# rapidsai/cugraph-gnn

Hardware: AMD Instinct MI355X
Metric: sampled-edges/sec (sample+renumber+feature-gather+SAGEConv fwd), ogbn-products-like fan-out [25, 10] (higher is better)
Workload: dtype int64 ids (int32 timed as a variant) + f32 features (SAGE lin_l/lin_r product: bf16x3-split MFMA, f32 accumulate); 1 GPU; ogbn-products-like RMAT: V=2449029, E=118462496 directed (CSR row_ptr i64 / col i64 replicated per GPU), feat fp32 [V,100], batch 1024/GPU, fan-out [25, 10], 2-layer SAGEConv(mean) 100-256-47 fwd, step = 8 call groups of 188 mini-batches; parallelism=dp1 (seeds sharded, no data-path collective)

## Files before the change

cugraph-gnn_amd/csrc/wg_rng.hpp:

```cpp
#pragma once
#include <hip/hip_runtime.h>

#include <cstdint>

namespace wgamd {

struct PcgJump {
  uint64_t a;
  uint64_t s;
};

struct PcgJumpTables {
  PcgJump t[4][256];
  constexpr PcgJumpTables() : t{}
  {
    uint64_t base_a = 6364136223846793005ULL, base_s = 1;
    for (int k = 0; k < 4; k++) {
      t[k][0].a = 1;
      t[k][0].s = 0;
      for (int c = 1; c < 256; c++) {
        t[k][c].a = t[k][c - 1].a * base_a;
        t[k][c].s = t[k][c - 1].s * base_a + base_s;
      }
      for (int d = 0; d < 8; d++) {
        uint64_t na = base_a * base_a, ns = base_s * base_a + base_s;
        base_a = na;
        base_s = ns;
      }
    }
  }
};

__device__ __constant__ const PcgJumpTables g_pcg_jump{};

struct Pcg32 {
  uint64_t state;
  uint64_t inc;

  static constexpr uint64_t kMult = 6364136223846793005ULL;

  __host__ __device__ __forceinline__ uint32_t next_u32()
  {
    uint64_t old = state;
    state        = old * kMult + inc;
    uint32_t x   = (uint32_t)(((old >> 18u) ^ old) >> 27u);
    uint32_t rot = (uint32_t)(old >> 59u);
    return (x >> rot) | (x << ((0u - rot) & 31u));
  }

  __host__ __device__ __forceinline__ void skipahead(uint64_t delta)
  {
    uint64_t acc_mult = 1u, acc_plus = 0u, cur_mult = kMult, cur_plus = inc;
    while (delta) {
      if (delta & 1u) {
        acc_mult *= cur_mult;
        acc_plus = acc_plus * cur_mult + cur_plus;
      }
      cur_plus = (cur_mult + 1u) * cur_plus;
      cur_mult *= cur_mult;
      delta >>= 1u;
    }
    state = acc_mult * state + acc_plus;
  }

  __host__ __device__ __forceinline__ Pcg32(uint64_t seed, uint64_t subsequence)
  {
    state = 0u;
    inc   = (subsequence << 1u) | 1u;
    (void)next_u32();
    state += seed;
    (void)next_u32();
    skipahead(subsequence);
  }

  __device__ __forceinline__ void jump_table(uint32_t n)
  {
    PcgJump j = g_pcg_jump.t[0][n & 255u];
#pragma unroll
    for (int k = 1; k < 4; k++) {
      const uint32_t c = (n >> (8 * k)) & 255u;
      if (c) {
        const PcgJump m = g_pcg_jump.t[k][c];
        j.s             = j.s * m.a + m.s;
        j.a             = j.a * m.a;
      }
    }
    state = j.a * state + inc * j.s;
  }

  struct table_tag {};
  __device__ __forceinline__ Pcg32(uint64_t seed, uint32_t subsequence, table_tag, uint32_t extra_draws = 0)
  {
    inc   = ((uint64_t)subsequence << 1u) | 1u;
    state = (inc + seed) * kMult + inc;
    jump_table(subsequence + extra_draws);
  }

  __host__ __device__ __forceinline__ int32_t next_i31() { return (int32_t)(next_u32() & 0x7fffffffu); }
  __host__ __device__ __forceinline__ uint64_t next_u64()
  {
    uint64_t lo = next_u32();
    uint64_t hi = next_u32();
    return lo | (hi << 32u);
  }
  __host__ __device__ __forceinline__ int64_t next_i63() { return (int64_t)(next_u64() & 0x7fffffffffffffffULL); }
  __host__ __device__ __forceinline__ float next_f32() { return (float)(next_u32() >> 8u) / 16777216.0f; }
};

}
```

cugraph-gnn_amd/csrc/wg_sample.hip:

```cpp
#include <algorithm>
#include <cmath>

#include "wg_common.hpp"
#include "wg_rng.hpp"

namespace wgamd {
namespace {

template <typename T>
struct dtype_of;
template <>
struct dtype_of<int32_t> {
  static constexpr wholememory_dtype_t value = WHOLEMEMORY_DT_INT;
};
template <>
struct dtype_of<int64_t> {
  static constexpr wholememory_dtype_t value = WHOLEMEMORY_DT_INT64;
};

__host__ __device__ constexpr int ref_block_threads(int M)
{
  int f = (M - 1) / 32;
  return f < 3 ? 32 : f < 6 ? 64 : f < 12 ? 128 : 256;
}
// ... 102 lines not shown

template <typename ColT>
__device__ __forceinline__ ColT col_at(const ColT* __restrict__ col, int64_t at)
{
  return col ? col[at] : (ColT)0;
}

constexpr int kWalkGrid = 256 * 16;

template <typename ColT>
__device__ __forceinline__ void emit(ColT* dst, int* src_lid, int64_t* edge_gid, int64_t out, ColT v,
                                     int seed_index, int64_t gid)
{
  if (dst) dst[out] = v;
  if (src_lid) src_lid[out] = seed_index;
  if (edge_gid) edge_gid[out] = gid;
}

struct loc_rec {
  int64_t start;
  int i;
  int deg;
  int base;
  int i_local;
  int batch;
  int pad;
};
static_assert(sizeof(loc_rec) == 32, "one 32-byte sector per record");
constexpr int kLocBuckets = 4096;
constexpr int kLocBlocks  = 128;
constexpr int kLocThreads = 1024;

template <typename SeedT>
__global__ void __launch_bounds__(kLocThreads)
locality_hist_kernel(const SeedT* __restrict__ seeds, dev_count n_, int shift, int* __restrict__ hist )
{
  __shared__ int h[kLocBuckets];
  const int n = n_.get(), per = (n + kLocBlocks - 1) / kLocBlocks;
  const int lo = min(n, (int)blockIdx.x * per), hi = min(n, lo + per);
  for (int k = threadIdx.x; k < kLocBuckets; k += kLocThreads) h[k] = 0;
  __syncthreads();
  for (int i = lo + threadIdx.x; i < hi; i += kLocThreads)
    atomicAdd(&h[min((int)((uint64_t)seeds[i] >> shift), kLocBuckets - 1)], 1);
  __syncthreads();
  for (int k = threadIdx.x; k < kLocBuckets; k += kLocThreads) hist[(int64_t)blockIdx.x * kLocBuckets + k] = h[k];
}

template <typename SeedT>
__global__ void __launch_bounds__(kLocThreads)
locality_scatter_kernel(const SeedT* __restrict__ seeds, dev_count n_, int shift, const int* __restrict__ hist,
                        const int64_t* __restrict__ row_start, const int* __restrict__ row_deg, const int* __restrict__ offsets,
                        rng_plan rng, loc_rec* __restrict__ recs)
{
  __shared__ int cursor[kLocBuckets];
  __shared__ int wave_tot[kLocThreads / 64];
  static_assert(kLocBuckets == 4 * kLocThreads, "thread t owns buckets 4 t .. 4 t + 3");
  const int n = n_.get(), per = (n + kLocBlocks - 1) / kLocBlocks;
  const int lo = min(n, (int)blockIdx.x * per), hi = min(n, lo + per);
  int tot[4] = {0, 0, 0, 0}, before[4] = {0, 0, 0, 0};
  const int4* h4 = reinterpret_cast<const int4*>(hist);
  for (int b = 0; b < kLocBlocks; b++) {
    const int4 v = h4[(int64_t)b * (kLocBuckets / 4) + threadIdx.x];
    tot[0] += v.x; tot[1] += v.y; tot[2] += v.z; tot[3] += v.w;
    if (b < (int)blockIdx.x) { before[0] += v.x; before[1] += v.y; before[2] += v.z; before[3] += v.w; }
  }
  const int sum = tot[0] + tot[1] + tot[2] + tot[3];
  int inc = sum;
  const int lane = threadIdx.x & 63, wave = threadIdx.x >> 6;
#pragma unroll
  for (int d = 1; d < 64; d <<= 1) {
    const int up = __shfl_up(inc, d, 64);
    if (lane >= d) inc += up;
  }
  if (lane == 63) wave_tot[wave] = inc;
  __syncthreads();
  int run = inc - sum;
  for (int w = 0; w < wave; w++) run += wave_tot[w];
#pragma unroll
  for (int k = 0; k < 4; k++) {
    cursor[4 * threadIdx.x + k] = run + before[k];
    run += tot[k];
  }
  __syncthreads();
  for (int i = lo + threadIdx.x; i < hi; i += kLocThreads) {
    const int j = atomicAdd(&cursor[min((int)((uint64_t)seeds[i] >> shift), kLocBuckets - 1)], 1);
    loc_rec r;
    r.start = row_start[i];
    r.i     = i;
    r.deg   = row_deg[i];
    r.base  = offsets[i];
    r.i_local = i;
    r.batch   = 0;
    if (rng.target_batch) {
      r.batch   = rng.target_batch[i];
      r.i_local = i - rng.target_seg[r.batch];
    }
    r.pad   = 0;
    recs[j] = r;
  }
}

template <typename SeedT, typename ColT, int LANES>
__global__ void __launch_bounds__(256) sample_uniform_halfwave_kernel(const int64_t* __restrict__ row_ptr,
                                                                      const ColT* __restrict__ col,
                                                                      const SeedT* __restrict__ seeds,
                                                                      dev_count n_,
                                                                      int M,
                                                                      rng_plan rng,
                                                                      const int* __restrict__ offsets,
                                                                      ColT* __restrict__ dst,
                                                                      int* __restrict__ src_lid,
                                                                      int64_t* __restrict__ edge_gid,
                                                                      const int64_t* __restrict__ row_start,
                                                                      const int* __restrict__ row_deg,
                                                                      const loc_rec* __restrict__ recs = nullptr)
{
  const int n    = n_.get();
  const int lane = threadIdx.x & 63;
  const int hl   = lane & (LANES - 1);
  const int hb   = lane & ~(LANES - 1);
  int i          = (int)(((int64_t)blockIdx.x * blockDim.x + threadIdx.x) / LANES);
  loc_rec rec{};
  if (recs) {
    constexpr int kGroups = 256 / LANES;
    const int per_x = ((n + 7) / 8 + kGroups - 1) / kGroups * kGroups;
    const int k     = (int)(blockIdx.x >> 3) * kGroups + (int)threadIdx.x / LANES;
    const int j     = (int)(blockIdx.x & 7) * per_x + k;
    i               = n;
    if (k < per_x && j < n) {
      rec = recs[j];
      i   = rec.i;
    }
  }
  int32_t r_draw = 0;
  if (i < n && hl < M) {
    uint64_t random_seed;
    int i_local;
    if (recs) {
      i_local     = rec.i_local;
      random_seed = rng.seeds_dev ? rng.seeds_dev[rec.batch] : rng.seed;
    } else
      rng.resolve(i, random_seed, i_local);
    if (i_local < (1 << 26)) {
      Pcg32 g(random_seed, (uint32_t)(i_local * 32 + hl), Pcg32::table_tag{});
      r_draw = g.next_i31();
    } else {
      Pcg32 g(random_seed, stream_id(i_local, 32, hl));
      r_draw = g.next_i31();
    }
  }
  int64_t start = 0;
  int N = 0, base = 0;
  if (i < n && recs) {
    start = rec.start;
    N     = rec.deg;
    base  = rec.base;
  } else if (i < n) {
    if (row_start) {
      start = row_start[i];
      N     = row_deg[i];
    } else {
      int64_t nid = (int64_t)seeds[i];
      start       = row_ptr[nid];
      N           = (int)(row_ptr[nid + 1] - start);
    }
    base = offsets[i];
  }
  const bool pick = N > M;
  if (__ballot(pick) == 0ull) {
    if (hl < N) emit<ColT>(dst, src_lid, edge_gid, (int64_t)base + hl, col_at<ColT>(col, start + hl), i, start + hl);
    return;
  }
  int r = 0;
  if (pick && hl < M) r = r_draw % (N - hl);
  const int tail = N - hl - 1;
  int p1 = -1, p2 = -1;
  for (int s = 0; s + 1 < M; s++) {
    const int rs    = __shfl(r, hb | s, 64);
    const bool prev = s < hl;
    p1 = (prev && rs == r) ? s : p1;
    p2 = (prev && rs == tail) ? s : p2;
  }
  int root = p2 >= 0 ? p2 : hl;
#pragma unroll
  for (int round = 0; round < (LANES == 32 ? 5 : 4); round++) root = __shfl(root, hb | root, 64);
  const int val = N - root - 1;
  const int vp1 = __shfl(val, hb | (p1 & (LANES - 1)), 64);
  const int a   = p1 >= 0 ? vp1 : r;
  if (pick) {
    if (hl < M) emit<ColT>(dst, src_lid, edge_gid, (int64_t)base + hl, col_at<ColT>(col, start + a), i, start + a);
  } else if (hl < N) {
    emit<ColT>(dst, src_lid, edge_gid, (int64_t)base + hl, col_at<ColT>(col, start + hl), i, start + hl);
  }
}

template <typename SeedT, typename ColT, int GW, int K, bool EXACT>
__global__ void __launch_bounds__(256)
sample_uniform_multi_kernel(const ColT* __restrict__ col, dev_count n_, int M_rt, rng_plan rng, const int* __restrict__ offsets,
                            ColT* __restrict__ dst, int* __restrict__ src_lid, int64_t* __restrict__ edge_gid,
                            const int64_t* __restrict__ row_start, const int* __restrict__ row_deg,
                            const loc_rec* __restrict__ recs)
{
  constexpr int kGPW    = 64 / GW;
  constexpr int kGroups = 4 * kGPW;
  constexpr int kRounds = GW <= 2 ? 1 : GW <= 4 ? 2 : GW <= 8 ? 3 : GW <= 16 ? 4 : 5;
  const int M    = EXACT ? GW : M_rt;
  const int n    = n_.get();
  const int lane = threadIdx.x & 63;
  const int grp  = lane / GW;
  const int hl   = lane - grp * GW;
  const int hb   = grp * GW;
  const bool live_group = grp < kGPW;
  const int wg_group    = (int)(threadIdx.x >> 6) * kGPW + grp;
  const int per_x = ((n + 7) / 8 + kGroups * K - 1) / (kGroups * K) * (kGroups * K);
  const int64_t n_chunks = recs ? (int64_t)(per_x / (kGroups * K)) * 8 : ((int64_t)n + kGroups * K - 1) / (kGroups * K);
  for (int64_t chunk = blockIdx.x; chunk < n_chunks; chunk += gridDim.x) {
  int i[K], N[K], base[K], i_local[K], batch[K];
  int64_t start[K];
  if (recs) {
    const int k0    = ((int)(chunk >> 3) * kGroups + wg_group) * K;
#pragma unroll
    for (int k = 0; k < K; k++) {
      const int j = (int)(chunk & 7) * per_x + k0 + k;
      i[k] = n, N[k] = 0, base[k] = 0, start[k] = 0, i_local[k] = 0, batch[k] = 0;
      if (live_group && k0 + k < per_x && j < n) {
        const loc_rec r = recs[j];
        i[k] = r.i, N[k] = r.deg, base[k] = r.base, start[k] = r.start, i_local[k] = r.i_local, batch[k] = r.batch;
      }
    }
  } else {
    const int64_t g = chunk * kGroups + wg_group;
#pragma unroll
    for (int k = 0; k < K; k++) {
      i[k] = live_group ? (int)min(g * K + k, (int64_t)n) : n;
      N[k] = 0, base[k] = 0, start[k] = 0, i_local[k] = i[k], batch[k] = 0;
      if (i[k] < n) {
        start[k] = row_start[i[k]];
        N[k]     = row_deg[i[k]];
        base[k]  = offsets[i[k]];
        if (rng.target_batch) batch[k] = rng.target_batch[i[k]];
      }
    }
    if (rng.target_batch) {
#pragma unroll
      for (int k = 0; k < K; k++)
        if (i[k] < n) i_local[k] = i[k] - rng.target_seg[batch[k]];
    }
  }
  int32_t r_draw[K];
#pragma unroll
  for (int k = 0; k < K; k++) {
    r_draw[k] = 0;
    if (i[k] < n && hl < M) {
      const uint64_t random_seed = rng.seeds_dev ? rng.seeds_dev[rng.target_batch ? batch[k] : 0] : rng.seed;
      if (i_local[k] < (1 << 26)) {
        Pcg32 g(random_seed, (uint32_t)(i_local[k] * 32 + hl), Pcg32::table_tag{});
        r_draw[k] = g.next_i31();
      } else {
        Pcg32 g(random_seed, stream_id(i_local[k], 32, hl));
        r_draw[k] = g.next_i31();
      }
    }
  }
  int a[K];
#pragma unroll
  for (int k = 0; k < K; k++) {
    const bool pick = N[k] > M;
    a[k]            = hl;
    if (__ballot(pick) != 0ull) {
      int r = 0;
      if (pick && hl < M) r = r_draw[k] % (N[k] - hl);
      const int tail = N[k] - hl - 1;
      int p1 = -1, p2 = -1;
      auto step = [&](int s) {
        const int rs    = __shfl(r, hb + s, 64);
        const bool prev = s < hl;
        p1 = (prev && rs == r) ? s : p1;
        p2 = (prev && rs == tail) ? s : p2;
      };
      if constexpr (EXACT) {
#pragma unroll
        for (int s = 0; s + 1 < GW; s++) step(s);
      } else {
        for (int s = 0; s + 1 < M; s++) step(s);
      }
      int root = p2 >= 0 ? p2 : hl;
#pragma unroll
      for (int round = 0; round < kRounds; round++) root = __shfl(root, hb + root, 64);
      const int val = N[k] - root - 1;
      const int vp1 = __shfl(val, hb + max(p1, 0), 64);
      if (pick) a[k] = p1 >= 0 ? vp1 : r;
    }
  }
  ColT v[K];
  bool on[K];
#pragma unroll
  for (int k = 0; k < K; k++) {
    on[k] = live_group && hl < (N[k] > M ? M : N[k]);
    v[k]  = on[k] ? col_at<ColT>(col, start[k] + a[k]) : (ColT)0;
  }
#pragma unroll
  for (int k = 0; k < K; k++)
    if (on[k]) emit<ColT>(dst, src_lid, edge_gid, (int64_t)base[k] + hl, v[k], i[k], start[k] + a[k]);
  }
}

constexpr int kHashSlots = 4096;

__device__ __forceinline__ int lds_hash_find(const int* keys, int pos)
{
  uint32_t h = ((uint32_t)pos * 2654435761u) & (kHashSlots - 1);
  while (true) {
    int k = keys[h];
    if (k == pos || k == -1) return (int)h;
    h = (h + 1) & (kHashSlots - 1);
  }
}

template <typename SeedT, typename ColT>
__global__ void __launch_bounds__(256) sample_uniform_block_kernel(const int64_t* __restrict__ row_ptr,
                                                                   const ColT* __restrict__ col,
                                                                   const SeedT* __restrict__ seeds,
                                                                   dev_count n_,
                                                                   int M,
                                                                   int B,
                                                                   int items,
                                                                   rng_plan rng,
                                                                   const int* __restrict__ offsets,
                                                                   ColT* __restrict__ dst,
                                                                   int* __restrict__ src_lid,
                                                                   int64_t* __restrict__ edge_gid)
{
  __shared__ int r[1024];
  __shared__ int a[1024];
  __shared__ int hkeys[kHashSlots];
  __shared__ int hvals[kHashSlots];
  const int i = blockIdx.x;
  if (i >= n_.get()) return;
  const int64_t nid   = (int64_t)seeds[i];
  const int64_t start = row_ptr[nid];
  const int N         = (int)(row_ptr[nid + 1] - start);
  if (N <= 0) return;
  const int base = offsets[i];
  if (N <= M) {
    for (int j = threadIdx.x; j < N; j += blockDim.x)
      emit<ColT>(dst, src_lid, edge_gid, (int64_t)base + j, col_at<ColT>(col, start + j), i, start + j);
    return;
  }
  for (int h = threadIdx.x; h < kHashSlots; h += blockDim.x) hkeys[h] = -1;
  if ((int)threadIdx.x < B) {
    uint64_t random_seed;
    int i_local;
    rng.resolve(i, random_seed, i_local);
    Pcg32 g(random_seed, stream_id(i_local, B, threadIdx.x));
    for (int k = 0; k < items; k++) {
      int id = k * B + threadIdx.x;
      int v  = g.next_i31();
      if (id < M) r[id] = v % (N - id);
    }
  }
  __syncthreads();
  if (threadIdx.x == 0) {
    for (int t = 0; t < M; t++) {
      const int rt = r[t], tail = N - t - 1;
      int s1     = lds_hash_find(hkeys, rt);
      int q_rt   = hkeys[s1] == rt ? hvals[s1] : rt;
      int s2     = lds_hash_find(hkeys, tail);
      int q_tail = hkeys[s2] == tail ? hvals[s2] : tail;
      a[t]       = q_rt;
      hkeys[s1]  = rt;
      hvals[s1]  = q_tail;
    }
  }
  __syncthreads();
  for (int t = threadIdx.x; t < M; t += blockDim.x)
    emit<ColT>(dst, src_lid, edge_gid, (int64_t)base + t, col_at<ColT>(col, start + a[t]), i, start + a[t]);
}

template <typename SeedT, typename ColT>
__global__ void __launch_bounds__(64) sample_uniform_reservoir_kernel(const int64_t* __restrict__ row_ptr,
                                                                      const ColT* __restrict__ col,
                                                                      const SeedT* __restrict__ seeds,
                                                                      dev_count n_,
                                                                      int M,
                                                                      rng_plan rng,
                                                                      const int* __restrict__ offsets,
                                                                      ColT* __restrict__ dst,
                                                                      int* __restrict__ src_lid,
                                                                      int64_t* __restrict__ edge_gid)
{
  const int i = blockIdx.x;
  if (i >= n_.get()) return;
  const int64_t nid   = (int64_t)seeds[i];
  const int64_t start = row_ptr[nid];
  const int N         = (int)(row_ptr[nid + 1] - start);
  if (N <= 0) return;
  const int64_t base = offsets[i];
  if (N <= M) {
    for (int j = threadIdx.x; j < N; j += blockDim.x)
      emit<ColT>(dst, src_lid, edge_gid, base + j, col_at<ColT>(col, start + j), i, start + j);
    return;
  }
  for (int s = threadIdx.x; s < M; s += blockDim.x) dst[base + s] = (ColT)s;
  __syncthreads();
  if (threadIdx.x < 32) {
    uint64_t random_seed;
    int i_local;
    rng.resolve(i, random_seed, i_local);
    Pcg32 g(random_seed, stream_id(i_local, 32, threadIdx.x));
    for (int idx = M + threadIdx.x; idx < N; idx += 32) {
      int rn = g.next_i31() % (idx + 1);
      if (rn < M) {
        if constexpr (sizeof(ColT) == 8)
          atomicMax(reinterpret_cast<long long*>(dst + base + rn), (long long)idx);
        else
          atomicMax(reinterpret_cast<int*>(dst + base + rn), idx);
      }
    }
  }
  __syncthreads();
  for (int s = threadIdx.x; s < M; s += blockDim.x) {
    int sel = (int)__hip_atomic_load(dst + base + s, __ATOMIC_RELAXED, __HIP_MEMORY_SCOPE_AGENT);
    emit<ColT>(dst, src_lid, edge_gid, base + s, col_at<ColT>(col, start + sel), i, start + sel);
  }
}

__device__ __forceinline__ float ares_key(float w, Pcg32& g, bool* redrawn = nullptr)
{
  float u = g.next_f32();
  u       = (float)(-(0.5 + 0.5 * (double)u));
  uint64_t x;
  int zero_draws = -1;
  do {
    x = g.next_u64();
    zero_draws++;
  } while (!x);
  if (redrawn != nullptr && zero_draws > 0) *redrawn = true;
  int one_bit = __clzll((long long)x) + zero_draws * 64;
  u *= exp2f((float)(-one_bit));
#ifdef WG_TUNE_CHEAP_KEY
  return u * 1.442695f * __builtin_amdgcn_rcpf(w);
#endif
  return (log1pf(u) / logf(2.0f)) * (1.0f / w);
}

constexpr int kWaveRowCap = 1024;
static_assert(kWaveRowCap == kWaveRowCapDecl, "keep the two in step");

__device__ __forceinline__ uint32_t key_bits(float k)
{
  uint32_t b = __float_as_uint(k);
  return (b & 0x80000000u) ? ~b : (b | 0x80000000u);
}

constexpr int kLdsKeys = kWeightedLdsKeys;

template <typename SeedT, typename ColT, typename WeightT, int B, int T>
__global__ void __launch_bounds__(T) sample_weighted_kernel(const int64_t* __restrict__ row_ptr,
                                                            const ColT* __restrict__ col,
                                                            const WeightT* __restrict__ weight,
                                                            const SeedT* __restrict__ seeds,
                                                            dev_count n_,
                                                            int M,
                                                            rng_plan rng,
                                                            const int* __restrict__ offsets,
                                                            uint32_t* __restrict__ slab,
                                                            int64_t slab_len,
                                                            ColT* __restrict__ dst,
                                                            int* __restrict__ src_lid,
                                                            int64_t* __restrict__ edge_gid,
                                                            int* __restrict__ lists ,
                                                            int list_cap,
                                                            int redo = 0 )
{
  static_assert(T % B == 0 && T % 64 == 0, "threads must be a multiple of the stream layout and of the wave");
  __shared__ uint32_t lds_keys[kLdsKeys];
  __shared__ int hist[256];
  __shared__ int sh_digit, sh_need, sh_redo;
  __shared__ int wave_cnt[2][T / 64];
  __shared__ int sh_li;
  const int n_live  = n_.get();
  const int n_huge  = lists && !redo ? lists[8] : 0;
  const int count   = lists ? (redo ? lists[kWeightedRedoCount] : n_huge + lists[7]) : n_live;
  uint32_t* gkeys   = slab + (int64_t)blockIdx.x * slab_len;
  int li            = blockIdx.x;
  while (true) {
  __syncthreads();
  if (lists) {
    if (threadIdx.x == 0) sh_li = atomicAdd(lists + (redo ? kWeightedRedoHead : 9), 1);
    __syncthreads();
    li = sh_li;
  }
  if (li >= count) break;
  const int i = lists ? (redo ? lists[kWeightedListHead + (int64_t)kWeightedRedoList * list_cap + li]
                         : li < n_huge ? lists[kWeightedListHead + 8 * (int64_t)list_cap + li]
                                       : lists[kWeightedListHead + 7 * (int64_t)list_cap + (li - n_huge)])
                      : li;
  if (!lists) li += gridDim.x;
  if (i >= n_live) continue;
  uint64_t random_seed;
  int i_rng;
  rng.resolve(i, random_seed, i_rng);
  const int64_t nid   = (int64_t)seeds[i];
  const int64_t start = row_ptr[nid];
  const int N         = (int)(row_ptr[nid + 1] - start);
  if (N <= 0) continue;
  const int64_t base = offsets[i];
  if (M <= 0 || N <= M) {
    for (int j = threadIdx.x; j < N; j += T)
      emit<ColT>(dst, src_lid, edge_gid, base + j, col_at<ColT>(col, start + j), i, start + j);
    continue;
  }
  const bool in_lds = N <= kLdsKeys;
  auto put = [&](int id, uint32_t k) { if (in_lds) lds_keys[id] = k; else gkeys[id] = k; };
  auto get = [&](int id) -> uint32_t {
    return in_lds ? lds_keys[id] : __hip_atomic_load(gkeys + id, __ATOMIC_RELAXED, __HIP_MEMORY_SCOPE_AGENT);
  };
  if (threadIdx.x == 0) sh_redo = 0;
  __syncthreads();
  {
    constexpr int hop = T / B;
    const int lane = threadIdx.x % B, part = threadIdx.x / B;
    const int L     = lane < N ? (N - lane + B - 1) / B : 0;
    const int share = (L + hop - 1) / hop;
    const int m0 = part * share, m1 = min(L, m0 + share);
    bool redrawn = false;
    if (m0 < m1) {
      const int64_t sid = (int64_t)i_rng * B + lane;
      Pcg32 g = (sid < (1ll << 31)) ? Pcg32(random_seed, (uint32_t)sid, Pcg32::table_tag{}, 3u * (uint32_t)m0)
                                    : Pcg32(random_seed, stream_id(i_rng, B, lane));
      if (sid >= (1ll << 31)) g.skipahead(3u * (uint64_t)m0);
      for (int m = m0; m < m1; m++) {
        const int id = lane + m * B;
        put(id, key_bits(ares_key((float)weight[start + id], g, &redrawn)));
      }
    }
    if (redrawn) sh_redo = 1;
  }
  __syncthreads();
  if (T > B && sh_redo) {
    if (threadIdx.x < B) {
      Pcg32 g = stream_generator(random_seed, i_rng, B, threadIdx.x);
      for (int id = threadIdx.x; id < N; id += B) put(id, key_bits(ares_key((float)weight[start + id], g)));
    }
    __syncthreads();
  }
  uint32_t prefix = 0, prefix_mask = 0;
  int need = M;
  for (int shift = 24; shift >= 0; shift -= 8) {
    for (int h = threadIdx.x; h < 256; h += T) hist[h] = 0;
    __syncthreads();
    for (int id = threadIdx.x; id < N; id += T) {
      uint32_t k = get(id);
      if ((k & prefix_mask) == prefix) atomicAdd(&hist[(k >> shift) & 255], 1);
    }
    __syncthreads();
    if (threadIdx.x < 64) {
      const int l  = threadIdx.x;
      const int h0 = hist[4 * l], h1 = hist[4 * l + 1], h2 = hist[4 * l + 2], h3 = hist[4 * l + 3];
      const int own = h0 + h1 + h2 + h3;
      int inc = own;
      for (int off = 1; off < 64; off <<= 1) {
        int v = __shfl_down(inc, off);
        if (l + off < 64) inc += v;
      }
      int acc = inc - own;
      if (acc < need && need <= inc) {
        int d = 4 * l + 3;
        if (acc + h3 < need) {
          acc += h3;
          d = 4 * l + 2;
          if (acc + h2 < need) {
            acc += h2;
            d = 4 * l + 1;
            if (acc + h1 < need) {
              acc += h1;
              d = 4 * l;
            }
          }
        }
        sh_digit = d;
        sh_need  = need - acc;
      }
    }
    __syncthreads();
    prefix |= (uint32_t)sh_digit << shift;
    prefix_mask |= 255u << shift;
    need = sh_need;
    __syncthreads();
  }
  const uint32_t thr = prefix;
  int out_run = 0, tie_run = 0;
  const int lane = threadIdx.x & 63, wave = threadIdx.x >> 6;
  for (int chunk = 0; chunk < N; chunk += T) {
    int id     = chunk + threadIdx.x;
    uint32_t k = id < N ? get(id) : 0u;
    bool gt    = id < N && k > thr;
    bool eq    = id < N && k == thr;
    uint64_t meq = __ballot(eq);
    int eq_before_in_wave = __popcll(meq & ((1ull << lane) - 1ull));
    if (lane == 0) wave_cnt[1][wave] = __popcll(meq);
    __syncthreads();
    int eq_before = tie_run + eq_before_in_wave, eq_total = 0;
    for (int w = 0; w < T / 64; w++) {
      if (w < wave) eq_before += wave_cnt[1][w];
      eq_total += wave_cnt[1][w];
// ... 392 lines not shown
  __shared__ float c_a[kCandCap];
  __shared__ uint32_t c_kb[kCandCap];
  __shared__ int hist[256];
  __shared__ int sh_li, sh_count, sh_rare, sh_digit, sh_need, sh_keep, sh_eq;
  __shared__ uint32_t sh_thr, sh_kmin, sh_sel[2];
  __shared__ uint32_t sh_wthr[W];
  __shared__ int keep_id[32], eq_id[kEqCap];
  __shared__ float keep_a[32], eq_a[kEqCap];
  const int tid = threadIdx.x, lane = tid & 63, wave = tid >> 6;
  const int n_live = n_.get();
  const int n_huge = lists[8];
  const int count  = n_huge + lists[7];

  auto append = [&](int id, float a) {
    const int p = atomicAdd(&sh_count, 1);
    if (p < kCandCap) {
      c_id[p] = id;
      c_a[p]  = a;
    } else {
      sh_rare = 1;
    }
  };

  while (true) {
    __syncthreads();
    if (tid == 0) sh_li = atomicAdd(lists + 9, 1);
    __syncthreads();
    const int li = sh_li;
    if (li >= count) break;
    const int i = li < n_huge ? lists[kWeightedListHead + 8 * (int64_t)list_cap + li]
                              : lists[kWeightedListHead + 7 * (int64_t)list_cap + (li - n_huge)];
    if (i >= n_live) continue;
    uint64_t random_seed;
    int i_rng;
    rng.resolve(i, random_seed, i_rng);
    const int64_t nid   = (int64_t)seeds[i];
    const int64_t start = row_ptr[nid];
    const int N         = (int)(row_ptr[nid + 1] - start);
    const int64_t base  = offsets[i];
    if (tid == 0) {
      sh_count = 0;
      sh_rare  = force_redo;
      sh_thr   = 0x7f800000u;
    }
    auto compress = [&](bool last) {
      __syncthreads();
      const int n = min(sh_count, kCandCap);
      for (int e = tid; e < n; e += T) c_kb[e] = key_bits(ares_key_exact(c_a[e], (float)weight[start + c_id[e]]));
      if (tid == 0) {
        sh_keep = 0;
        sh_eq   = 0;
        sh_kmin = ~0u;
      }
      __syncthreads();
      uint32_t prefix = 0u, hi = 0u;
      int need = M;
      if (n <= 256) {
        if (wave == 0) {
          uint32_t kb[4];
#pragma unroll
          for (int j = 0; j < 4; j++) kb[j] = lane + 64 * j < n ? c_kb[lane + 64 * j] : 0u;
          int match = n;
#pragma unroll 1
          for (int bit = 31; bit >= 0 && match != need; bit--) {
            const uint32_t cand = prefix | (1u << bit);
            hi |= 1u << bit;
            int cnt = 0;
#pragma unroll
            for (int j = 0; j < 4; j++) cnt += __popcll(__ballot(kb[j] != 0u && (kb[j] & hi) == cand));
            if (cnt >= need) {
              prefix = cand;
              match  = cnt;
            } else {
              need -= cnt;
              match -= cnt;
            }
          }
          if (lane == 0) {
            sh_sel[0] = prefix;
            sh_sel[1] = hi;
            sh_need   = need;
          }
        }
        __syncthreads();
        prefix = sh_sel[0];
        hi     = sh_sel[1];
        need   = sh_need;
      } else {
        for (int shift = 24; shift >= 0; shift -= 8) {
          for (int h = tid; h < 256; h += T) hist[h] = 0;
          __syncthreads();
          for (int e = tid; e < n; e += T) {
            const uint32_t kk = c_kb[e];
            if ((kk & hi) == prefix) atomicAdd(&hist[(kk >> shift) & 255], 1);
          }
          __syncthreads();
          if (tid < 64) {
            const int l  = tid;
            const int h0 = hist[4 * l], h1 = hist[4 * l + 1], h2 = hist[4 * l + 2], h3 = hist[4 * l + 3];
            const int own = h0 + h1 + h2 + h3;
            int inc = own;
            for (int off = 1; off < 64; off <<= 1) {
              int v = __shfl_down(inc, off);
              if (l + off < 64) inc += v;
            }
            int acc = inc - own;
            if (acc < need && need <= inc) {
              int d = 4 * l + 3;
              if (acc + h3 < need) {
                acc += h3;
                d = 4 * l + 2;
                if (acc + h2 < need) {
                  acc += h2;
                  d = 4 * l + 1;
                  if (acc + h1 < need) {
                    acc += h1;
                    d = 4 * l;
                  }
                }
              }
              sh_digit = d;
              sh_need  = need - acc;
            }
          }
          __syncthreads();
          prefix |= (uint32_t)sh_digit << shift;
          hi |= 255u << shift;
          need = sh_need;
          __syncthreads();
        }
      }
      for (int e = tid; e < n; e += T) {
        const uint32_t kk = c_kb[e], kd = kk & hi;
        if (kk != 0u && kd > prefix) {
          const int p = atomicAdd(&sh_keep, 1);
          keep_id[p]  = c_id[e];
          keep_a[p]   = c_a[e];
          atomicMin(&sh_kmin, kk);
        } else if (kk != 0u && kd == prefix) {
          const int q = atomicAdd(&sh_eq, 1);
          if (q < kEqCap) {
            eq_id[q] = c_id[e];
            eq_a[q]  = c_a[e];
            atomicMin(&sh_kmin, kk);
          } else {
            sh_rare = 1;
          }
        }
      }
      __syncthreads();
      const int eqc = min(sh_eq, kEqCap);
      if (tid < eqc) {
        int rank = 0;
        for (int j = 0; j < eqc; j++) rank += eq_id[j] < eq_id[tid] ? 1 : 0;
        if (rank < need) {
          const int p = atomicAdd(&sh_keep, 1);
          keep_id[p]  = eq_id[tid];
          keep_a[p]   = eq_a[tid];
        }
      }
      __syncthreads();
      if (last) {
        if (tid < M && !sh_rare) {
          const int mine = keep_id[tid];
          int rank = 0;
          for (int j = 0; j < M; j++) rank += keep_id[j] < mine ? 1 : 0;
          emit<ColT>(dst, src_lid, edge_gid, base + rank, col_at<ColT>(col, start + mine), i, start + mine);
        }
      } else {
        if (tid < M) {
          c_id[tid] = keep_id[tid];
          c_a[tid]  = keep_a[tid];
        }
        if (tid == 0) {
          sh_count = M;
          sh_thr   = (~sh_kmin) & 0x7fffffffu;
        }
      }
      __syncthreads();
    };

    const int sl = tid % B, part = tid / B;
    const int L     = (N - sl + B - 1) / B;
    const int share = (L + 3) / 4;
    const int m0 = part * share, m1 = min(L, m0 + share);
    const int rounds = (((N + B - 1) / B) + 3) / 4;
    const int64_t sid = (int64_t)i_rng * B + sl;
    Pcg32 g0 = (sid < (1ll << 31)) ? Pcg32(random_seed, (uint32_t)sid, Pcg32::table_tag{}, 3u * (uint32_t)m0)
                                   : Pcg32(random_seed, stream_id(i_rng, B, sl));
    if (sid >= (1ll << 31)) g0.skipahead(3u * (uint64_t)m0);
    KeyStream g(g0);
    bool rare = false;
    auto next = [&](float w, float& a, uint32_t& k) {
      a = g.next_mag(rare);
      rare |= weight_is_odd(w);
      k = __float_as_uint(a * __builtin_amdgcn_rcpf(w) * kMagScale);
    };
    auto weight_of = [&](int m) { return (float)weight[start + sl + (int64_t)min(m, m1 - 1) * B]; };
    const bool has0 = m0 < m1;
    float a0    = 0.f;
    uint32_t k0 = ~0u;
    if (has0) next(weight_of(m0), a0, k0);
    {
      const int nvalid = __popcll(__ballot(has0));
      uint32_t v = 0x7f800000u;
      if (nvalid >= M) {
        uint32_t prefix = 0u, hi = 0u;
        int need = M, match = nvalid;
#pragma unroll 1
        for (int bit = 31; bit >= 0 && match != need; bit--) {
          hi |= 1u << bit;
          const int cnt0 = __popcll(__ballot(has0 && (k0 & hi) == prefix));
          if (cnt0 >= need) {
            match = cnt0;
          } else {
            need -= cnt0;
            match -= cnt0;
            prefix |= 1u << bit;
          }
        }
        v = prefix | ~hi;
      }
      if (lane == 0) sh_wthr[wave] = v;
    }
    __syncthreads();
    uint32_t thr0 = sh_wthr[0];
#pragma unroll
    for (int w = 1; w < W; w++) thr0 = min(thr0, sh_wthr[w]);
    if (has0 && k0 <= thr0) append(m0 * B + sl, a0);
    compress(false);
    uint32_t thr = sh_thr;
    if (has0 && k0 > thr0 && k0 <= thr) append(m0 * B + sl, a0);
    for (int r = 1; r < rounds;) {
      if (__syncthreads_or(sh_count > kCandCap / 2)) compress(false);
      thr = sh_thr;
      float wv[kChunkRounds];
#pragma unroll
      for (int c = 0; c < kChunkRounds; c++) wv[c] = weight_of(m0 + r + c);
#pragma unroll
      for (int c = 0; c < kChunkRounds; c++) {
        const int m = m0 + r + c;
        if (m < m1) {
          float a;
          uint32_t k;
          next(wv[c], a, k);
          if (k <= thr) append(m * B + sl, a);
        }
      }
      r += kChunkRounds;
    }
    if (rare) sh_rare = 1;
    compress(true);
    if (tid == 0 && sh_rare) redo_append(lists, list_cap, i);
  }
}

template <typename SeedT, typename ColT>
__global__ void __launch_bounds__(256) copy_short_rows_kernel(const int64_t* __restrict__ row_ptr, const ColT* __restrict__ col,
                                                              const SeedT* __restrict__ seeds, dev_count n_, int M,
                                                              const int* __restrict__ offsets, ColT* __restrict__ dst,
                                                              int* __restrict__ src_lid, int64_t* __restrict__ edge_gid)
{
  const int64_t t = (int64_t)blockIdx.x * blockDim.x + threadIdx.x;
  const int i = (int)(t >> 4), hl = (int)(t & 15);
  if (i >= n_.get()) return;
  const int64_t nid   = (int64_t)seeds[i];
  const int64_t start = row_ptr[nid];
  const int N         = (int)(row_ptr[nid + 1] - start);
  if (N <= 0 || N > M) return;
  const int64_t base = offsets[i];
  for (int j = hl; j < N; j += 16) emit<ColT>(dst, src_lid, edge_gid, base + j, col_at<ColT>(col, start + j), i, start + j);
}

template <typename SeedT, typename ColT>
void uniform_launch(const int64_t* row_ptr, const ColT* col, const SeedT* seeds, dev_count n, int M,
                    rng_plan random_seed, const int* offsets, ColT* dst, int* lid, int64_t* gid, hipStream_t stream,
                    const int64_t* row_start = nullptr, const int* row_deg = nullptr, const sample_locality* loc = nullptr)
{
  const int cap = n.host;
  if (cap <= 0) return;
  if (M > 0 && M <= 32 && row_start != nullptr) {
    static const int K = [] {
      const char* e = getenv("WGAMD_SAMPLE_K");
      const int k   = e ? atoi(e) : 4;
      return k == 1 || k == 2 ? k : 4;
    }();
    const loc_rec* recs = nullptr;
    if (loc != nullptr) {
      auto* r = static_cast<loc_rec*>(loc->recs);
      locality_hist_kernel<SeedT><<<kLocBlocks, kLocThreads, 0, stream>>>(seeds, n, loc->shift, loc->hist);
      locality_scatter_kernel<SeedT><<<kLocBlocks, kLocThreads, 0, stream>>>(seeds, n, loc->shift, loc->hist, row_start, row_deg,
                                                                            offsets, random_seed, r);
      recs = r;
    }
#define WG_MULTI(GW, KK)                                                                                             \
  sample_uniform_multi_kernel<SeedT, ColT, GW, KK, WG_EXACT>                                                          \
    <<<(int)std::min<int64_t>((ceil_div((int64_t)cap, 4 * (64 / GW) * KK) + 15) / 8 * 8, kWalkGrid), 256, 0, stream>>>(           \
      col, n, M, random_seed, offsets, dst, lid, gid, row_start, row_deg, recs)
#define WG_MULTI_K(GW)                                                                                               \
  do {                                                                                                               \
    if (K == 1) WG_MULTI(GW, 1); else if (K == 2) WG_MULTI(GW, 2); else WG_MULTI(GW, 4);                              \
  } while (0)
    static const bool exact = getenv("WGAMD_SAMPLE_EXACT_WIDTH") == nullptr || atoi(getenv("WGAMD_SAMPLE_EXACT_WIDTH")) != 0;
#define WG_EXACT true
    if (exact && M == 5) WG_MULTI_K(5);
    else if (exact && M == 10) WG_MULTI_K(10);
    else if (exact && M == 15) WG_MULTI_K(15);
    else if (exact && M == 25) WG_MULTI_K(25);
    else {
#undef WG_EXACT
#define WG_EXACT false
      if (M <= 8) WG_MULTI_K(8);
      else if (M <= 16) WG_MULTI_K(16);
      else WG_MULTI_K(32);
    }
#undef WG_EXACT
#undef WG_MULTI_K
#undef WG_MULTI
    WG_HIP_CHECK(hipGetLastError());
    return;
  }
  if (M <= 0) {
    sample_uniform_block_kernel<SeedT, ColT><<<cap, 64, 0, stream>>>(row_ptr, col, seeds, n, 0x7fffffff, 32, 1,
                                                                     random_seed, offsets, dst, lid, gid);
  } else if (M <= 16) {
    sample_uniform_halfwave_kernel<SeedT, ColT, 16><<<ceil_div((int64_t)cap * 16, 256), 256, 0, stream>>>(
      row_ptr, col, seeds, n, M, random_seed, offsets, dst, lid, gid, row_start, row_deg);
  } else if (M <= 32) {
    sample_uniform_halfwave_kernel<SeedT, ColT, 32><<<ceil_div((int64_t)cap * 32, 256), 256, 0, stream>>>(
      row_ptr, col, seeds, n, M, random_seed, offsets, dst, lid, gid, row_start, row_deg);
  } else if (M <= 1024) {
    const int B = ref_block_threads(M);
    sample_uniform_block_kernel<SeedT, ColT><<<cap, B < 64 ? 64 : B, 0, stream>>>(
      row_ptr, col, seeds, n, M, B, ref_items_per_thread(M), random_seed, offsets, dst, lid, gid);
  } else {
    sample_uniform_reservoir_kernel<SeedT, ColT><<<cap, 64, 0, stream>>>(row_ptr, col, seeds, n, M, random_seed,
                                                                         offsets, dst, lid, gid);
  }
  WG_HIP_CHECK(hipGetLastError());
}

inline int& weighted_mode(int which)
{
  static int mode[2] = {[] { const char* e = getenv("WGAMD_WEIGHTED_PRUNING"); return e && e[0] == '0' ? 0 : 1; }(),
                        [] { const char* e = getenv("WGAMD_WEIGHTED_FORCE_REDO"); return e && e[0] == '1' ? 1 : 0; }()};
  return mode[which];
}
inline bool weighted_pruning_off() { return weighted_mode(0) == 0; }
inline int weighted_force_redo() { return weighted_mode(1); }

struct side_stream {
  int device         = -1;
  hipStream_t stream = nullptr;
  hipEvent_t fork = nullptr, join = nullptr;
  void ensure()
  {
    int dev = 0;
    WG_HIP_CHECK(hipGetDevice(&dev));
    if (stream != nullptr && dev == device) return;
    device = dev;
    WG_HIP_CHECK(hipStreamCreateWithFlags(&stream, hipStreamNonBlocking));
    WG_HIP_CHECK(hipEventCreateWithFlags(&fork, hipEventDisableTiming));
    WG_HIP_CHECK(hipEventCreateWithFlags(&join, hipEventDisableTiming));
  }
};
inline side_stream& weighted_side_stream()
{
  static thread_local side_stream s;
  s.ensure();
  return s;
}

template <typename SeedT, typename ColT, typename WeightT>
void weighted_sample_launch(const int64_t* row_ptr, const ColT* col, const WeightT* weights, const SeedT* seeds, dev_count n,
                            int M, rng_plan rng, const int* offsets, int* lists, int blocks, uint32_t* slab,
                            int64_t slab_len, ColT* dst, int* lid, int64_t* gid, hipStream_t stream)
{
  if (n.host <= 0) return;
  const int cap = n.host;
  if (M <= 0 || M > 256) {
    sample_weighted_kernel<SeedT, ColT, WeightT, 256, 256><<<std::max(blocks, 1), 256, 0, stream>>>(
      row_ptr, col, weights, seeds, n, M, rng, offsets, slab, slab_len, dst, lid, gid, nullptr, 0);
    return;
  }
  const bool pruned = M <= 32 && !weighted_pruning_off();
  bool forked = false;
  side_stream* side = nullptr;
  if (blocks > 0 && pruned) {
    side = &weighted_side_stream();
    WG_HIP_CHECK(hipEventRecord(side->fork, stream));
    WG_HIP_CHECK(hipStreamWaitEvent(side->stream, side->fork, 0));
    sample_weighted_block_pruned_kernel<SeedT, ColT, WeightT><<<blocks, 512, 0, side->stream>>>(
      row_ptr, col, weights, seeds, n, M, rng, offsets, dst, lid, gid, lists, cap, weighted_force_redo());
    WG_HIP_CHECK(hipEventRecord(side->join, side->stream));
    forked = true;
  } else if (blocks > 0)
    sample_weighted_kernel<SeedT, ColT, WeightT, 128, 512><<<blocks, 512, 0, stream>>>(
      row_ptr, col, weights, seeds, n, M, rng, offsets, slab, slab_len, dst, lid, gid, lists, cap);
  if (M < 16)
    sample_weighted_group_kernel<SeedT, ColT, WeightT, 16><<<ceil_div((int64_t)cap * 16, 256), 256, 0, stream>>>(
      row_ptr, col, weights, seeds, M, rng, offsets, dst, lid, gid, lists, cap, 0);
  if (M < 32)
    sample_weighted_group_kernel<SeedT, ColT, WeightT, 32><<<ceil_div((int64_t)cap * 32, 256), 256, 0, stream>>>(
      row_ptr, col, weights, seeds, M, rng, offsets, dst, lid, gid, lists, cap, 1);
  if (M < 64)
    sample_weighted_group_kernel<SeedT, ColT, WeightT, 64><<<ceil_div((int64_t)cap * 64, 256), 256, 0, stream>>>(
      row_ptr, col, weights, seeds, M, rng, offsets, dst, lid, gid, lists, cap, 2);
#define WG_WAVE(KM, CLS)                                                                                               \
  do {                                                                                                                 \
    if (pruned)                                                                                                        \
      sample_weighted_wave_pruned_kernel<SeedT, ColT, WeightT, KM><<<ceil_div(cap, 4), 256, 0, stream>>>(              \
        row_ptr, col, weights, seeds, M, rng, offsets, dst, lid, gid, lists, cap, CLS, weighted_force_redo());          \
    else                                                                                                               \
      sample_weighted_wave_kernel<SeedT, ColT, WeightT, KM><<<ceil_div(cap, 4), 256, 0, stream>>>(                     \
        row_ptr, col, weights, seeds, M, rng, offsets, dst, lid, gid, lists, cap, CLS);                                \
  } while (0)
  if (M < 128) WG_WAVE(2, 3);
  WG_WAVE(4, 4);
  WG_WAVE(8, 5);
  WG_WAVE(16, 6);
#undef WG_WAVE
  copy_short_rows_kernel<SeedT, ColT><<<ceil_div((int64_t)cap * 16, 256), 256, 0, stream>>>(row_ptr, col, seeds, n, M, offsets,
                                                                                          dst, lid, gid);
  if (forked) WG_HIP_CHECK(hipStreamWaitEvent(stream, side->join, 0));
  if (pruned)
    sample_weighted_kernel<SeedT, ColT, WeightT, 128, 512><<<blocks > 0 ? std::min(blocks, 128) : 64, 512, 0, stream>>>(
      row_ptr, col, weights, seeds, n, M, rng, offsets, slab, slab_len, dst, lid, gid, lists, cap, 1);
}

struct sample_args {
  wholememory_tensor_t row_ptr, col, weight, seeds, out_offsets;
  int M;
  void *dst_ctx, *lid_ctx, *gid_ctx;
  uint64_t random_seed;
  wholememory_env_func_t* env;
  hipStream_t stream;
};

void validate(const sample_args& a, bool weighted)
{
  WG_REQUIRE_INPUT(a.row_ptr && a.col && a.seeds && a.out_offsets && a.env, "null tensor / env");
  WG_REQUIRE_INPUT(a.dst_ctx != nullptr, "output_dest_memory_context must not be NULL");
  auto rd = a.row_ptr->desc, cd = a.col->desc, sd = a.seeds->desc, od = a.out_offsets->desc;
  WG_REQUIRE_INPUT(rd.dim == 1 && cd.dim == 1 && sd.dim == 1 && od.dim == 1, "all tensors must be 1-D");
  WG_REQUIRE_INPUT(!weighted || (!a.row_ptr->handle && !a.col->handle),
                   "weighted sampling needs CSR tensors that wrap device pointers (a partitioned CSR is served for the "
                   "unweighted op only, as in the reference)");
  WG_EXPECTS(rd.dtype == WHOLEMEMORY_DT_INT64, "csr_row_ptr dtype must be INT64, got %d", (int)rd.dtype);
  WG_EXPECTS(od.dtype == WHOLEMEMORY_DT_INT, "output_sample_offset dtype must be INT, got %d", (int)od.dtype);
  WG_REQUIRE_INPUT(cd.dtype == WHOLEMEMORY_DT_INT || cd.dtype == WHOLEMEMORY_DT_INT64, "csr_col dtype must be INT|INT64");
  WG_REQUIRE_INPUT(sd.dtype == WHOLEMEMORY_DT_INT || sd.dtype == WHOLEMEMORY_DT_INT64, "center_nodes dtype must be INT|INT64");
  WG_REQUIRE_INPUT(od.sizes[0] == sd.sizes[0] + 1, "output_sample_offset must have center_node_count+1 entries");
  WG_REQUIRE_INPUT(sd.sizes[0] < (int64_t)1 << 31, "too many center nodes");
  if (weighted) {
    WG_REQUIRE_INPUT(a.weight && !a.weight->handle && a.weight->desc.dim == 1, "csr_weight must be a 1-D device tensor");
    WG_REQUIRE_INPUT(a.weight->desc.dtype == WHOLEMEMORY_DT_FLOAT || a.weight->desc.dtype == WHOLEMEMORY_DT_DOUBLE,
                     "csr_weight dtype must be FLOAT|DOUBLE");
    WG_REQUIRE_INPUT(a.weight->desc.sizes[0] == cd.sizes[0], "csr_weight and csr_col sizes differ");
  }
}

template <typename SeedT>
__global__ void __launch_bounds__(256)
max_degree_kernel(const int64_t* __restrict__ row_ptr, const SeedT* __restrict__ seeds, int n, int threshold, int* __restrict__ out)
{
  const int i = blockIdx.x * blockDim.x + threadIdx.x;
  if (i >= n) return;
  const int64_t nid = (int64_t)seeds[i];
  const int deg     = (int)(row_ptr[nid + 1] - row_ptr[nid]);
  if (deg > threshold) atomicMax(out, deg);
}

template <typename SeedT, typename ColT, typename WeightT>
void run(const sample_args& a, bool weighted)
{
  const int n            = (int)a.seeds->desc.sizes[0];
  const int M            = a.M;
  hipStream_t stream     = a.stream;
  const auto* row_ptr    = static_cast<const int64_t*>(tensor_data(a.row_ptr));
  const auto* col        = static_cast<const ColT*>(tensor_data(a.col));
  const auto* seeds      = static_cast<const SeedT*>(tensor_data(a.seeds));
  int* offsets           = static_cast<int*>(tensor_data(a.out_offsets));
  const WeightT* weights = weighted ? static_cast<const WeightT*>(tensor_data(a.weight)) : nullptr;

  temp_buffer cnt_buf(a.env), scan_tmp(a.env), list_buf(a.env);
  int* cnt  = cnt_buf.device<int>(n + 1, WHOLEMEMORY_DT_INT);
  int* stmp = scan_tmp.device<int>(scan_tmp_ints(n + 1), WHOLEMEMORY_DT_INT);
  const bool wave_path = weighted && M > 0 && M <= 256;
  int* big_list        = weighted ? list_buf.device<int>(weighted_list_ints(n), WHOLEMEMORY_DT_INT) : nullptr;
  int h_tot[3]         = {0, 0, 0};
  int h_head[kWeightedListHead] = {0};

  if (weighted) {
    WG_HIP_CHECK(hipMemsetAsync(big_list, 0, kWeightedListHead * sizeof(int), stream));
    if (n > 0 && wave_path)
      sample_count_kernel<SeedT><<<ceil_div(n, 256), 256, 0, stream>>>(row_ptr, seeds, dev_count{n, nullptr}, M, cnt, nullptr,
                                                                      big_list, n, kLdsKeys);
    else if (n > 0)
      sample_count_kernel<SeedT><<<ceil_div(n, 256), 256, 0, stream>>>(row_ptr, seeds, dev_count{n, nullptr}, M, cnt, nullptr);
    WG_HIP_CHECK(hipGetLastError());
    WG_HIP_CHECK(hipMemcpyAsync(h_head, big_list, kWeightedListHead * sizeof(int), hipMemcpyDeviceToHost, stream));
  } else {
    sample_count_enqueue(row_ptr, seeds, sizeof(SeedT) == 8, dev_count{n, nullptr}, M, cnt, nullptr, stream);
  }
  exclusive_scan_i32(cnt, offsets, n, stmp, stream);
  WG_HIP_CHECK(hipMemcpyAsync(&h_tot[0], offsets + n, sizeof(int), hipMemcpyDeviceToHost, stream));
  WG_HIP_CHECK(hipStreamSynchronize(stream));
  const int total = h_tot[0];
  h_tot[1]        = h_head[7] + h_head[8];
  h_tot[2]        = h_head[10];
  if (weighted && !wave_path) {
    h_tot[2] = 0;
    if (n > 0) {
      temp_buffer deg_buf(a.env);
      int* dmax = deg_buf.device<int>(1, WHOLEMEMORY_DT_INT);
      WG_HIP_CHECK(hipMemsetAsync(dmax, 0, sizeof(int), stream));
      max_degree_kernel<SeedT><<<ceil_div(n, 256), 256, 0, stream>>>(row_ptr, seeds, n, kLdsKeys, dmax);
      WG_HIP_CHECK(hipMemcpyAsync(&h_tot[2], dmax, sizeof(int), hipMemcpyDeviceToHost, stream));
      WG_HIP_CHECK(hipStreamSynchronize(stream));
    }
  }

  auto* dst = static_cast<ColT*>(output_alloc(a.env, a.dst_ctx, total, dtype_of<ColT>::value));
  int* lid  = a.lid_ctx ? static_cast<int*>(output_alloc(a.env, a.lid_ctx, total, WHOLEMEMORY_DT_INT)) : nullptr;
  auto* gid = a.gid_ctx ? static_cast<int64_t*>(output_alloc(a.env, a.gid_ctx, total, WHOLEMEMORY_DT_INT64)) : nullptr;
  if (n == 0 || total == 0) return;

  if (weighted) {
    const int rows_for_blocks = wave_path ? h_tot[1] : n;
    const int blocks          = std::min(rows_for_blocks, kWeightedBlocks);
    const int64_t slab_len    = std::max(h_tot[2], 1);
    temp_buffer key_buf(a.env);
    uint32_t* slab = key_buf.device<uint32_t>(h_tot[2] > 0 ? (int64_t)blocks * slab_len : 1, WHOLEMEMORY_DT_INT);
    weighted_sample_launch<SeedT, ColT, WeightT>(row_ptr, col, weights, seeds, dev_count{n, nullptr}, M,
                                                 rng_plan{a.random_seed, nullptr, nullptr, nullptr}, offsets, big_list, blocks,
                                                 slab, slab_len, dst, lid, gid, stream);
    WG_HIP_CHECK(hipGetLastError());
    WG_HIP_CHECK(hipStreamSynchronize(stream));
    return;
  }
  uniform_sample_enqueue(row_ptr, col, sizeof(ColT) == 8, seeds, sizeof(SeedT) == 8, dev_count{n, nullptr}, M,
                         rng_plan{a.random_seed, nullptr, nullptr, nullptr}, offsets, dst, lid, gid, stream);
  WG_HIP_CHECK(hipGetLastError());
  WG_HIP_CHECK(hipStreamSynchronize(stream));
}

__global__ void __launch_bounds__(256) centre_pairs_kernel(const void* __restrict__ seeds, bool seeds64, int n,
                                                           int64_t* __restrict__ ids, int* __restrict__ twice)
{
  const int i = blockIdx.x * blockDim.x + threadIdx.x;
  if (i >= n) return;
  const int64_t v = seeds64 ? static_cast<const int64_t*>(seeds)[i] : (int64_t)static_cast<const int32_t*>(seeds)[i];
  ids[2 * i]     = v;
  ids[2 * i + 1] = v + 1;
  twice[i]       = 2 * i;
}

struct borrowed_tensor {
  wholememory_tensor_t t = nullptr;
  borrowed_tensor(void* p, int64_t n, wholememory_dtype_t dt)
  {
    wholememory_tensor_description_t d;
    wholememory_initialize_tensor_desc(&d);
    d.dim        = 1;
    d.dtype      = dt;
    d.sizes[0]   = n;
    d.strides[0] = 1;
    WG_EXPECTS(wholememory_make_tensor_from_pointer(&t, p, &d) == WHOLEMEMORY_SUCCESS, "tensor over scratch");
  }
  ~borrowed_tensor() { wholememory_destroy_tensor(t); }
  borrowed_tensor(const borrowed_tensor&)            = delete;
  borrowed_tensor& operator=(const borrowed_tensor&) = delete;
};

template <typename ColT>
void run_partitioned(const sample_args& a)
{
  const int n        = (int)a.seeds->desc.sizes[0];
  const int M        = a.M;
  hipStream_t stream = a.stream;
  const bool seeds64 = a.seeds->desc.dtype == WHOLEMEMORY_DT_INT64;
  int* offsets       = static_cast<int*>(tensor_data(a.out_offsets));
  auto fetch = [&](wholememory_tensor_t table, wholememory_tensor_t idx, wholememory_tensor_t out, const char* what) {
    const auto rc = wholememory_gather(table, idx, out, a.env, stream, -1);
    if (rc != WHOLEMEMORY_SUCCESS) throw logic_error(fmt("gather of %s failed (%d)", what, (int)rc));
  };
  temp_arena arena(a.env);
  const size_t o_ids = arena.add(sizeof(int64_t) * 2 * n), o_ptr = arena.add(sizeof(int64_t) * 2 * n),
               o_twice = arena.add(sizeof(int) * n), o_cnt = arena.add(sizeof(int) * (n + 1)),
               o_scan = arena.add(sizeof(int) * scan_tmp_ints(n + 1));
  arena.commit();
  int64_t* ids  = arena.at<int64_t>(o_ids);
  int64_t* ptrs = arena.at<int64_t>(o_ptr);
  int* twice    = arena.at<int>(o_twice);
  int* cnt      = arena.at<int>(o_cnt);
  if (n > 0) {
    centre_pairs_kernel<<<ceil_div(n, 256), 256, 0, stream>>>(tensor_data(a.seeds), seeds64, n, ids, twice);
    WG_HIP_CHECK(hipGetLastError());
  }
  {
    borrowed_tensor t_ids(ids, 2 * (int64_t)n, WHOLEMEMORY_DT_INT64), t_ptrs(ptrs, 2 * (int64_t)n, WHOLEMEMORY_DT_INT64);
    fetch(a.row_ptr, t_ids.t, t_ptrs.t, "csr_row_ptr");
  }
  sample_count_enqueue(ptrs, twice, false, dev_count{n, nullptr}, M, cnt, nullptr, stream);
  exclusive_scan_i32(cnt, offsets, n, arena.at<int>(o_scan), stream);
  int total = 0;
  WG_HIP_CHECK(hipMemcpyAsync(&total, offsets + n, sizeof(int), hipMemcpyDeviceToHost, stream));
  WG_HIP_CHECK(hipStreamSynchronize(stream));
  auto* dst = static_cast<ColT*>(output_alloc(a.env, a.dst_ctx, total, dtype_of<ColT>::value));
  int* lid  = a.lid_ctx ? static_cast<int*>(output_alloc(a.env, a.lid_ctx, total, WHOLEMEMORY_DT_INT)) : nullptr;
  temp_buffer gid_buf(a.env);
  auto* gid = a.gid_ctx ? static_cast<int64_t*>(output_alloc(a.env, a.gid_ctx, total, WHOLEMEMORY_DT_INT64))
                        : gid_buf.device<int64_t>(total, WHOLEMEMORY_DT_INT64);
  if (n > 0 && total > 0)
    uniform_sample_enqueue(ptrs, nullptr, sizeof(ColT) == 8, twice, false, dev_count{n, nullptr}, M,
                           rng_plan{a.random_seed, nullptr, nullptr, nullptr}, offsets, nullptr, lid, gid, stream);
  {
    borrowed_tensor t_gid(gid, total, WHOLEMEMORY_DT_INT64), t_dst(dst, total, dtype_of<ColT>::value);
    fetch(a.col, t_gid.t, t_dst.t, "csr_col");
  }
  WG_HIP_CHECK(hipStreamSynchronize(stream));
// ... 192 lines not shown
```

Measured before the change: 5.575 billion sampled-edges/s.

## Add one-seed-per-lane sampling kernel with LDS-compacted coalesced gather

Adds a sampling kernel in which each lane handles one seed and draws its M samples sequentially using a register-resident sparse Fisher-Yates swap map. The per-seed high part of the PCG jump is computed once and reused across draws. Picked offsets are then compacted through LDS so the wave gathers col entries and writes outputs contiguously. The aim is to cut the cross-lane shuffle work and the repeated jump-table cost of the group-per-seed multi kernel. The trade-off is more registers and LDS per thread for M=25, which may lower occupancy. The new kernel is used for exact widths when no locality records are present.

Result: faster. 5.685 billion sampled-edges/s, median of 6 (+2.0%).

```diff
diff --git a/cugraph-gnn_amd/csrc/wg_rng.hpp b/cugraph-gnn_amd/csrc/wg_rng.hpp
--- a/cugraph-gnn_amd/csrc/wg_rng.hpp
+++ b/cugraph-gnn_amd/csrc/wg_rng.hpp
@@ -96,6 +96,31 @@
     jump_table(subsequence + extra_draws);
   }
 
+  static __device__ __forceinline__ PcgJump jump_high(uint32_t n)
+  {
+    PcgJump h = g_pcg_jump.t[1][(n >> 8) & 255u];
+#pragma unroll
+    for (int k = 2; k < 4; k++) {
+      const uint32_t c = (n >> (8 * k)) & 255u;
+      if (c) {
+        const PcgJump m = g_pcg_jump.t[k][c];
+        h.s             = h.s * m.a + m.s;
+        h.a             = h.a * m.a;
+      }
+    }
+    return h;
+  }
+  struct split_tag {};
+  __device__ __forceinline__ Pcg32(uint64_t seed, uint32_t subsequence, split_tag, const PcgJump& high)
+  {
+    inc       = ((uint64_t)subsequence << 1u) | 1u;
+    state     = (inc + seed) * kMult + inc;
+    PcgJump j = g_pcg_jump.t[0][subsequence & 255u];
+    j.s       = j.s * high.a + high.s;
+    j.a       = j.a * high.a;
+    state     = j.a * state + inc * j.s;
+  }
+
   __host__ __device__ __forceinline__ int32_t next_i31() { return (int32_t)(next_u32() & 0x7fffffffu); }
   __host__ __device__ __forceinline__ uint64_t next_u64()
   {
diff --git a/cugraph-gnn_amd/csrc/wg_sample.hip b/cugraph-gnn_amd/csrc/wg_sample.hip
--- a/cugraph-gnn_amd/csrc/wg_sample.hip
+++ b/cugraph-gnn_amd/csrc/wg_sample.hip
@@ -428,6 +428,102 @@
 #pragma unroll
   for (int k = 0; k < K; k++)
     if (on[k]) emit<ColT>(dst, src_lid, edge_gid, (int64_t)base[k] + hl, v[k], i[k], start[k] + a[k]);
+  }
+}
+
+template <typename SeedT, typename ColT, int M>
+__global__ void __launch_bounds__(256)
+sample_uniform_lane_kernel(const ColT* __restrict__ col, dev_count n_, rng_plan rng, const int* __restrict__ offsets,
+                           ColT* __restrict__ dst, int* __restrict__ src_lid, int64_t* __restrict__ edge_gid,
+                           const int64_t* __restrict__ row_start, const int* __restrict__ row_deg)
+{
+  const int n    = n_.get();
+  const int lane = threadIdx.x & 63;
+  for (int64_t w = ((int64_t)blockIdx.x * 4 + (threadIdx.x >> 6)) * 64; w < n; w += (int64_t)gridDim.x * 256) {
+    const int i = (int)min(w + lane, (int64_t)n);
+    int N = 0, base = 0, batch = 0, i_local = i;
+    int64_t start = 0;
+    if (i < n) {
+      start = row_start[i];
+      N     = row_deg[i];
+      base  = offsets[i];
+      if (rng.target_batch) {
+        batch   = rng.target_batch[i];
+        i_local = i - rng.target_seg[batch];
+      }
+    }
+    int a[M];
+#pragma unroll
+    for (int t = 0; t < M; t++) a[t] = t;
+    const bool pick = N > M;
+    if (__ballot(pick) != 0ull && pick) {
+      const uint64_t random_seed = rng.seeds_dev ? rng.seeds_dev[rng.target_batch ? batch : 0] : rng.seed;
+      const bool tabled          = i_local < (1 << 26);
+      PcgJump high{1, 0};
+      if (tabled) high = Pcg32::jump_high((uint32_t)i_local * 32u);
+      int pos[M], val[M];
+#pragma unroll
+      for (int t = 0; t < M; t++) {
+        uint32_t r;
+        if (tabled) {
+          Pcg32 g(random_seed, (uint32_t)i_local * 32u + t, Pcg32::split_tag{}, high);
+          r = (uint32_t)g.next_i31();
+        } else {
+          Pcg32 g(random_seed, stream_id(i_local, 32, t));
+          r = (uint32_t)g.next_i31();
+        }
+        const int j    = (int)(r % (uint32_t)(N - t));
+        const int tail = N - t - 1;
+        int at_j = j, at_tail = tail;
+#pragma unroll
+        for (int s = 0; s < t; s++) {
+          at_j    = pos[s] == j ? val[s] : at_j;
+          at_tail = pos[s] == tail ? val[s] : at_tail;
+        }
+        a[t]   = at_j;
+        pos[t] = j;
+        val[t] = at_tail;
+      }
+    }
+    const int cnt = N > M ? M : N;
+    __shared__ int s_a[4][64 * M];
+    __shared__ unsigned char s_l[4][64 * M];
+    __shared__ int64_t s_start[4][64];
+    const int wv    = threadIdx.x >> 6;
+    const int last  = (int)min((int64_t)63, (int64_t)n - 1 - w);
+    const int wbase = __shfl(base, 0, 64);
+    const int total = min(__shfl(base + cnt, last, 64) - wbase, 64 * M);
+    const int rel   = base - wbase;
+    s_start[wv][lane] = start;
+#pragma unroll
+    for (int t = 0; t < M; t++)
+      if (t < cnt && (unsigned)(rel + t) < 64u * M) {
+        s_a[wv][rel + t] = a[t];
+        s_l[wv][rel + t] = (unsigned char)lane;
+      }
+    __builtin_amdgcn_fence(__ATOMIC_RELEASE, "wavefront");
+    __builtin_amdgcn_wave_barrier();
+    __builtin_amdgcn_fence(__ATOMIC_ACQUIRE, "wavefront");
+    int64_t at[M];
+    int owner[M];
+    ColT v[M];
+#pragma unroll
+    for (int k = 0; k < M; k++) {
+      const int idx = k * 64 + lane;
+      owner[k] = 0, at[k] = 0, v[k] = (ColT)0;
+      if (idx < total) {
+        owner[k] = s_l[wv][idx] & 63;
+        at[k]    = s_start[wv][owner[k]] + s_a[wv][idx];
+        v[k]     = col_at<ColT>(col, at[k]);
+      }
+    }
+#pragma unroll
+    for (int k = 0; k < M; k++) {
+      const int idx = k * 64 + lane;
+      if (idx < total) emit<ColT>(dst, src_lid, edge_gid, (int64_t)wbase + idx, v[k], (int)w + owner[k], at[k]);
+    }
+    __builtin_amdgcn_fence(__ATOMIC_RELEASE, "wavefront");
+    __builtin_amdgcn_wave_barrier();
   }
 }
 
@@ -1426,6 +1522,16 @@
     if (K == 1) WG_MULTI(GW, 1); else if (K == 2) WG_MULTI(GW, 2); else WG_MULTI(GW, 4);                              \
   } while (0)
     static const bool exact = getenv("WGAMD_SAMPLE_EXACT_WIDTH") == nullptr || atoi(getenv("WGAMD_SAMPLE_EXACT_WIDTH")) != 0;
+#define WG_LANE(MM)                                                                                                   \
+  sample_uniform_lane_kernel<SeedT, ColT, MM>                                                                         \
+    <<<(int)std::min<int64_t>(ceil_div((int64_t)cap, 256), kWalkGrid), 256, 0, stream>>>(col, n, random_seed, offsets, dst, lid, \
+                                                                                         gid, row_start, row_deg)
+    const bool lane_layout = exact && recs == nullptr;
+    if (lane_layout && M == 5) WG_LANE(5);
+    else if (lane_layout && M == 10) WG_LANE(10);
+    else if (lane_layout && M == 15) WG_LANE(15);
+    else if (lane_layout && M == 25) WG_LANE(25);
+    else
 #define WG_EXACT true
     if (exact && M == 5) WG_MULTI_K(5);
     else if (exact && M == 10) WG_MULTI_K(10);
@@ -1441,6 +1547,7 @@
 #undef WG_EXACT
 #undef WG_MULTI_K
 #undef WG_MULTI
+#undef WG_LANE
     WG_HIP_CHECK(hipGetLastError());
     return;
   }
```
